# Corv/CUDA-GMM-MPI

Hardware: NVIDIA H100
Metric: EM iterations/sec at N=10M D=24 K=64; E-step HBM GB/s vs roofline (higher is better)
Workload: dtype f32

## Files before the change

cuda-gmm-mpi_b200/csrc/kernels_tc.cu:

```cuda
#include <cuda.h>
#include <cudaTypedefs.h>
#include <cuda_fp16.h>
#if defined(__F16C__) && defined(__AVX__)
#include <immintrin.h>
#endif
#include <cuda_runtime.h>

#include <cmath>
#include <cstdio>
#include <cstdlib>
#include <cstring>
#include <string>
#include <vector>

#include "host_math.h"
#include "kernels_tc.cuh"
#include "mstep_rows.h"
#include "tc_ptx.cuh"

namespace gmm {

using namespace ptx;

#define TC_CUDA_TRY(expr)                                                                     \
    do {                                                                                      \
        cudaError_t e_ = (expr);                                                              \
        if (e_ != cudaSuccess)                                                                \
            return fail(GMM_ERR_CUDA, std::string(#expr) + ": " + cudaGetErrorString(e_));    \
    } while (0)

constexpr int kTE = 32;
constexpr int kNCL = 32;
constexpr int kNST = 3;
constexpr int kNRAW = 4;
constexpr int kChunkSub = 4;
constexpr int kChunkSub2 = 16;
constexpr int kPhiBits = 11;
constexpr float kGammaScale = 1024.0f;
constexpr float kGammaMagic = 1.5f * 134217728.0f;

template <int D> struct MCfg {
    static_assert(D % 4 == 0, "tensor M-step: D must be a multiple of 4");
    static constexpr int F = 1 + D + D * (D + 1) / 2;
    static constexpr int S = D / 4;
    static constexpr int MT = (4 * ((1 + 2 * S + S * (D / 2) + 7) / 8) * 8 + 127) / 128;
    static constexpr int G_PART = kNCL * kTE * 2;
    static constexpr int G_STAGE = 3 * G_PART;
    static constexpr int RAWZ = (D * kTE * 4 + 1023) / 1024 * 1024;
    static constexpr int RAWX = RAWZ + 1024;
    static constexpr int RAWG = kNCL * kTE * 4;
    static constexpr int OFF_G = 0;
    static constexpr int OFF_RAWX = OFF_G + kNST * G_STAGE;
    static constexpr int OFF_RAWG = OFF_RAWX + kNRAW * RAWX;
    static constexpr int NCT = MT * 128;
    static constexpr int OFF_RACC = OFF_RAWG + kNRAW * RAWG;
    static constexpr int OFF_BAR = OFF_RACC + 32 * NCT * 4;
    static constexpr int SMEM_BYTES = OFF_BAR + 512;
    static constexpr int THREADS = 128 + NCT;
    static constexpr int REG_LAUNCH = (65536 / THREADS) / 8 * 8 > 255 ? 255 : (65536 / THREADS) / 8 * 8;
    static constexpr int REG_P = MT == 1 ? REG_LAUNCH : 56;
    static constexpr int REG_C = MT == 3 ? 152 : (MT == 2 ? 224 : REG_LAUNCH);
    static_assert(128 * REG_P + NCT * REG_C <= THREADS * REG_LAUNCH, "register pools");
    static_assert(OFF_RAWX % 1024 == 0 && RAWX % 1024 == 0 && RAWZ % 1024 == 0, "SWIZZLE_128B TMA destinations need 1024-byte alignment");
    static_assert(OFF_RAWG % 1024 == 0 && RAWG % 1024 == 0, "SWIZZLE_128B TMA destinations need 1024-byte alignment");
    static_assert(MT <= 3, "feature tiles");
};

template <int R, int L>
__device__ __forceinline__ void set_regs() {
    if constexpr (R < L) asm volatile("setmaxnreg.dec.sync.aligned.u32 %0;" ::"n"(R));
    else if constexpr (R > L) asm volatile("setmaxnreg.inc.sync.aligned.u32 %0;" ::"n"(R));
}

struct MMagic { float lin, prod; };

__device__ __forceinline__ void tma_load_2d(void* smem_dst, const CUtensorMap* tmap, int c0, int c1, uint64_t* bar) {
    asm volatile(
        "cp.async.bulk.tensor.2d.shared::cluster.global.mbarrier::complete_tx::bytes [%0], [%1, {%2, %3}], [%4];"
        ::"r"(smem_u32(smem_dst)), "l"(reinterpret_cast<uint64_t>(tmap)), "r"(c0), "r"(c1), "r"(smem_u32(bar)) : "memory");
}

__device__ __forceinline__ float2 lds_f2(uint32_t addr) {
    float2 v;
    asm volatile("ld.shared.v2.f32 {%0, %1}, [%2];" : "=f"(v.x), "=f"(v.y) : "r"(addr) : "memory");
    return v;
}

__device__ __forceinline__ void feature_split(float a, float b, float m, float& h, float& l) {
    h = __fsub_rn(__fmaf_rn(a, b, m), m);
    l = __fmaf_rn(a, b, -h);
}

#ifndef GMM_MSTEP_CUT
#define GMM_MSTEP_CUT 0
#endif

__device__ __forceinline__ void build_half(const float2 (&za)[4], const float2 (&zb0)[4], const float2 (&zb1)[4], float m0, float m1,
                                           uint32_t (&hi)[2][4], uint32_t (&lo)[2][4]) {
#pragma unroll
    for (int p = 0; p < 4; p++) {
        const int ks = p >> 1, u = p & 1;
#if GMM_MSTEP_CUT == 2
        hi[ks][2 * u] = __float_as_uint(zb0[p].x); hi[ks][2 * u + 1] = __float_as_uint(zb1[p].x);
        lo[ks][2 * u] = __float_as_uint(zb0[p].y); lo[ks][2 * u + 1] = __float_as_uint(zb1[p].y);
        (void)za; (void)m0; (void)m1;
#else
        float h0, l0, h1, l1, h2, l2, h3, l3;
        feature_split(za[p].x, zb0[p].x, m0, h0, l0);
        feature_split(za[p].y, zb0[p].y, m0, h1, l1);
        feature_split(za[p].x, zb1[p].x, m1, h2, l2);
        feature_split(za[p].y, zb1[p].y, m1, h3, l3);
        hi[ks][2 * u] = pack_half2(h0, h1);
        hi[ks][2 * u + 1] = pack_half2(h2, h3);
        lo[ks][2 * u] = pack_half2(l0, l1);
        lo[ks][2 * u + 1] = pack_half2(l2, l3);
#endif
    }
}

__device__ __forceinline__ void load_row(uint32_t addr, float2 (&z)[4]) {
#pragma unroll
    for (int p = 0; p < 4; p++) z[p] = lds_f2(addr ^ (uint32_t)(p << 5));
}

__device__ __forceinline__ void issue_half(float (&ex)[16], float (&rm)[16], const uint32_t (&hi)[2][4], const uint32_t (&lo)[2][4],
                                           uint32_t gam, bool new1, bool new2) {
#pragma unroll
    for (int ks = 0; ks < kTE / 16; ks++) {
        const uint64_t hdesc = make_smem_desc(gam + ks * 256,  128,  512);
        const uint64_t ldesc = make_smem_desc(gam + kNCL * kTE * 2 + ks * 256, 128, 512);
        const uint64_t sdesc = make_smem_desc(gam + 2 * kNCL * kTE * 2 + ks * 256, 128, 512);
#if GMM_MSTEP_CUT == 1
        asm volatile("" ::"r"(hi[ks][0]), "r"(hi[ks][1]), "r"(hi[ks][2]), "r"(hi[ks][3]), "r"(lo[ks][0]), "r"(lo[ks][1]), "r"(lo[ks][2]),
                     "r"(lo[ks][3]), "l"(hdesc), "l"(ldesc), "l"(sdesc));
        (void)ex; (void)rm; (void)new1; (void)new2;
#else
        wgmma_m64n32k16_rs(ex, hi[ks][0], hi[ks][1], hi[ks][2], hi[ks][3], hdesc, ks > 0 || !new1);
        wgmma_m64n32k16_rs(rm, hi[ks][0], hi[ks][1], hi[ks][2], hi[ks][3], ldesc, ks > 0 || !new2);
        wgmma_m64n32k16_rs(rm, lo[ks][0], lo[ks][1], lo[ks][2], lo[ks][3], sdesc, true);
#endif
    }
}

__device__ __forceinline__ bool chain_ends(int i, int mt, int nsub) { return ((i + mt) % kChunkSub) == kChunkSub - 1 || i == nsub - 1; }
__device__ __forceinline__ bool chain_starts(int i, int mt) { return i == 0 || ((i + mt) % kChunkSub) == 0; }
__device__ __forceinline__ bool chain2_ends(int i, int mt, int nsub) { return ((i + mt) % kChunkSub2) == kChunkSub2 - 1 || i == nsub - 1; }
__device__ __forceinline__ bool chain2_starts(int i, int mt) { return i == 0 || ((i + mt) % kChunkSub2) == 0; }

template <int D>
__global__ void __launch_bounds__(MCfg<D>::THREADS, 1)
mstep_tc_kernel(const __grid_constant__ CUtensorMap tm_x, const __grid_constant__ CUtensorMap tm_g, int n,
                float* __restrict__ scratch, int events_per_cta, const __grid_constant__ MMagic magic, const int* __restrict__ opmap) {
    using C = MCfg<D>;
    extern __shared__ __align__(1024) uint8_t smem[];
    uint64_t* bars = reinterpret_cast<uint64_t*>(smem + C::OFF_BAR);
    uint64_t* raw_full = bars;
    uint64_t* raw_empty = bars + kNRAW;
    uint64_t* op_full = bars + 2 * kNRAW;
    uint64_t* op_empty = op_full + kNST;

    const int warp = threadIdx.x >> 5, lane = threadIdx.x & 31;
    const int e_begin = blockIdx.x * events_per_cta;
    const int e_end = min(n, e_begin + events_per_cta);
    const int nsub = (e_end - e_begin + kTE - 1) / kTE;
    const int k0 = blockIdx.y * kNCL;

    for (int i = threadIdx.x; i < kNRAW * 256; i += C::THREADS)
        reinterpret_cast<float*>(smem + C::OFF_RAWX + (i >> 8) * C::RAWX + C::RAWZ)[i & 255] = 1.0f;
    if (threadIdx.x == 0) {
        for (int s = 0; s < kNRAW; s++) { mbar_init(&raw_full[s], 1); mbar_init(&raw_empty[s], 3 + 4 * C::MT); }
        for (int s = 0; s < kNST; s++) { mbar_init(&op_full[s], 3); mbar_init(&op_empty[s], 4 * C::MT); }
        fence_mbar_init();
    }
    __syncthreads();

    if (warp < 4) {
        set_regs<C::REG_P, C::REG_LAUNCH>();
        if (warp == 0) {
            if (elect_one()) {
                for (int i = 0; i < nsub; i++) {
                    const int st = i % kNRAW, ph = (i / kNRAW) & 1;
                    mbar_wait_parked(&raw_empty[st], ph ^ 1, 500);
                    mbar_arrive_expect_tx(&raw_full[st], kTE * D * 4 + C::RAWG);
                    const int e0 = e_begin + i * kTE;
                    tma_load_2d(smem + C::OFF_RAWX + st * C::RAWX, &tm_x, e0, 0, &raw_full[st]);
                    tma_load_2d(smem + C::OFF_RAWG + st * C::RAWG, &tm_g, e0, k0, &raw_full[st]);
                }
            }
        } else {
            const int bt = threadIdx.x - 32;
            constexpr int NIT = 2;
            for (int i = 0; i < nsub; i++) {
                const int rs = i % kNRAW, rph = (i / kNRAW) & 1;
                const int os = i % kNST, oph = (i / kNST) & 1;
                mbar_wait_parked(&raw_full[rs], rph, 200);
                uint4 gh[NIT], gl[NIT], gs[NIT];
                float dep = 0.0f;
#pragma unroll
                for (int u = 0; u < NIT; u++) {
                    const int it = bt + 96 * u;
                    if (it >= 128) break;
                    const int kg = it >> 5, l = it & 31;
                    const int k = kg * 8 + (l & 7), ce = l >> 3;
                    const uint8_t* grow = smem + C::OFF_RAWG + rs * C::RAWG + k * (kTE * 4);
                    const float4 a = *reinterpret_cast<const float4*>(grow + (((2 * ce) ^ (k & 7)) << 4));
                    const float4 b = *reinterpret_cast<const float4*>(grow + (((2 * ce + 1) ^ (k & 7)) << 4));
                    const float g[8] = {a.x, a.y, a.z, a.w, b.x, b.y, b.z, b.w};
                    dep += a.x + b.x;
                    float hi[8], lo[8];
#pragma unroll
                    for (int v = 0; v < 8; v++) {
                        hi[v] = __fsub_rn(__fmaf_rn(g[v], kGammaScale, kGammaMagic), kGammaMagic);
                        lo[v] = __fmaf_rn(g[v], kGammaScale, -hi[v]);
                    }
                    gh[u] = make_uint4(pack_half2(hi[0], hi[1]), pack_half2(hi[2], hi[3]), pack_half2(hi[4], hi[5]), pack_half2(hi[6], hi[7]));
                    gl[u] = make_uint4(pack_half2(lo[0], lo[1]), pack_half2(lo[2], lo[3]), pack_half2(lo[4], lo[5]), pack_half2(lo[6], lo[7]));
                    gs[u] = make_uint4(pack_half2(g[0] * kGammaScale, g[1] * kGammaScale), pack_half2(g[2] * kGammaScale, g[3] * kGammaScale),
                                       pack_half2(g[4] * kGammaScale, g[5] * kGammaScale), pack_half2(g[6] * kGammaScale, g[7] * kGammaScale));
                }
                __syncwarp();
                if (lane == 0) mbar_arrive_after(&raw_empty[rs], dep);
                else asm volatile("" ::"f"(dep));
                mbar_wait_parked(&op_empty[os], oph ^ 1, 200);
                uint8_t* g_hi = smem + C::OFF_G + os * C::G_STAGE;
#pragma unroll
                for (int u = 0; u < NIT; u++) {
                    const int it = bt + 96 * u;
                    if (it >= 128) break;
                    const int kg = it >> 5, l = it & 31;
                    *reinterpret_cast<uint4*>(g_hi + kg * 512 + l * 16) = gh[u];
                    *reinterpret_cast<uint4*>(g_hi + C::G_PART + kg * 512 + l * 16) = gl[u];
                    *reinterpret_cast<uint4*>(g_hi + 2 * C::G_PART + kg * 512 + l * 16) = gs[u];
                }
                fence_proxy_async_smem();
                __syncwarp();
                if (lane == 0) mbar_arrive(&op_full[os]);
            }
        }
    } else {
        set_regs<C::REG_C, C::REG_LAUNCH>();
        const int mt = __shfl_sync(0xffffffffu, (warp - 4) >> 2, 0);
        const int ct = threadIdx.x - 128;
        const int wq = warp & 3, gid = lane >> 2, qd = lane & 3;
        float* racc = reinterpret_cast<float*>(smem + C::OFF_RACC) + ct;
#pragma unroll
        for (int j = 0; j < 32; j++) racc[j * C::NCT] = 0.0f;
        uint32_t fa, fb[4];
        float mg[4];
        {
            const int* om = opmap + mt * 128 + wq * 16 + gid;
            auto addr = [&](int code) {
                const uint32_t row = code >= kRowOne ? (uint32_t)(C::RAWZ / 128 + code - kRowOne) : (uint32_t)code;
                return row * 128 + ((((uint32_t)qd >> 1) ^ (row & 7)) << 4) + ((uint32_t)qd & 1) * 8;
            };
#pragma unroll
            for (int s = 0; s < 4; s++) {
                const int c = om[(s >> 1) * 64 + (s & 1) * 8];
                const int a = c & 255, b = c >> 8;
                if (s == 0) fa = addr(a);
                fb[s] = addr(b);
                mg[s] = a >= kRowOne && b >= kRowOne ? 0.0f : (a >= kRowOne || b >= kRowOne ? magic.lin : magic.prod);
            }
        }
        const uint32_t zs0 = smem_u32(smem + C::OFF_RAWX);
        float ex[2][16], rm[2][16];
#pragma unroll
        for (int h = 0; h < 2; h++)
#pragma unroll
            for (int j = 0; j < 16; j++) { ex[h][j] = 0.0f; rm[h][j] = 0.0f; }
        uint32_t fh[2][2][4], fl[2][2][4];
        int held = -1;
        for (int i = 0; i < nsub; i++) {
            const int rs = i % kNRAW, rph = (i / kNRAW) & 1;
            const int os = i % kNST, oph = (i / kNST) & 1;
            const uint32_t zst = zs0 + rs * C::RAWX;
            const uint32_t gam = smem_u32(smem + C::OFF_G + os * C::G_STAGE);
            const bool new1 = chain_starts(i, mt), new2 = chain2_starts(i, mt);
            mbar_wait_parked(&raw_full[rs], rph, 100);
            float2 za[4], zb0[4], zb1[4];
            load_row(zst + fa, za);
            load_row(zst + fb[0], zb0);
            load_row(zst + fb[1], zb1);
            build_half(za, zb0, zb1, mg[0], mg[1], fh[0], fl[0]);
            mbar_wait_parked(&op_full[os], oph, 100);
            wgmma_fence();
            issue_half(ex[0], rm[0], fh[0], fl[0], gam, new1, new2);
            wgmma_commit();
            wgmma_wait<1>();
            __syncwarp();
            if (lane == 0 && held >= 0) mbar_arrive(&op_empty[held]);
            load_row(zst + fb[2], zb0);
            load_row(zst + fb[3], zb1);
            build_half(za, zb0, zb1, mg[2], mg[3], fh[1], fl[1]);
            wgmma_fence();
            issue_half(ex[1], rm[1], fh[1], fl[1], gam, new1, new2);
            wgmma_commit();
            __syncwarp();
            if (lane == 0) mbar_arrive(&raw_empty[rs]);
            wgmma_wait<1>();
            held = os;
            if (chain_ends(i, mt, nsub)) {
                wgmma_wait<0>();
                __syncwarp();
                if (lane == 0) mbar_arrive(&op_empty[os]);
                held = -1;
#if GMM_MSTEP_CUT != 3
#pragma unroll
                for (int h = 0; h < 2; h++) {
#pragma unroll
                    for (int j = 0; j < 16; j++) racc[(h * 16 + j) * C::NCT] += ex[h][j];
                    asm volatile("" ::: "memory");
                }
                if (chain2_ends(i, mt, nsub)) {
#pragma unroll
                    for (int h = 0; h < 2; h++) {
#pragma unroll
                        for (int j = 0; j < 16; j++) racc[(h * 16 + j) * C::NCT] += rm[h][j];
                        asm volatile("" ::: "memory");
                    }
                }
#endif
            }
        }
        wgmma_wait<0>();
#if GMM_MSTEP_CUT == 3
#pragma unroll
        for (int h = 0; h < 2; h++)
#pragma unroll
            for (int j = 0; j < 16; j++) racc[(h * 16 + j) * C::NCT] += ex[h][j] + rm[h][j];
#endif
        float* my = scratch + (size_t)(blockIdx.y * gridDim.x + blockIdx.x) * C::MT * 128 * kNCL + (size_t)mt * 128 * kNCL;
#pragma unroll
        for (int h = 0; h < 2; h++)
#pragma unroll
            for (int j = 0; j < 16; j += 2) {
                const int row = h * 64 + wq * 16 + gid + 8 * ((j >> 1) & 1);
                const int col = (j >> 2) * 8 + 2 * qd;
                *reinterpret_cast<float2*>(my + (size_t)row * kNCL + col) =
                    make_float2(racc[(h * 16 + j) * C::NCT], racc[(h * 16 + j + 1) * C::NCT]);
            }
    }
}

__global__ void standardise_soa_kernel(const float* __restrict__ xs, float* __restrict__ zs, size_t pitch, int n, int D,
                                       const float* __restrict__ shift_f, const float* __restrict__ inv_scale_f) {
    const int d = blockIdx.y;
    const float s = shift_f[d], isc = inv_scale_f[d];
    const float* x = xs + (size_t)d * pitch;
    float* z = zs + (size_t)d * pitch;
    for (long long e = (long long)blockIdx.x * blockDim.x + threadIdx.x; e < n; e += (long long)gridDim.x * blockDim.x)
        z[e] = __fmul_rn(__fsub_rn(x[e], s), isc);
}

__global__ void __launch_bounds__(256)
mstep_tc_finalize_kernel(const float* __restrict__ scratch, int ncta_x, int MT, int K, int F, const int3* __restrict__ rowmap,
                         const double* __restrict__ scale, double* __restrict__ stats) {
    constexpr int NQ = 256 / kNCL;
    __shared__ double part[NQ][kNCL];
    const int3 rm = rowmap[blockIdx.x];
    if (rm.x < 0) return;
    const int mt = blockIdx.x / 128, row = blockIdx.x % 128;
    const int col = threadIdx.x & (kNCL - 1), q = threadIdx.x / kNCL;
    double fac = 1.0 / (double)kGammaScale;
    if (rm.y >= 0) fac *= scale[rm.y];
    if (rm.z >= 0) fac *= scale[rm.z];
    for (int ty = 0; ty * kNCL < K; ty++) {
        double s = 0;
        for (int cx = q; cx < ncta_x; cx += NQ)
            s += (double)scratch[(((size_t)(ty * ncta_x + cx) * MT + mt) * 128 + row) * kNCL + col];
        part[q][col] = s;
        __syncthreads();
        const int k = ty * kNCL + col;
        if (q == 0 && k < K) {
            double t = 0;
#pragma unroll
            for (int u = 0; u < NQ; u++) t += part[u][col];
            stats[(size_t)k * F + rm.x] += t * fac;
        }
        __syncthreads();
    }
}


template <int D> struct ECfg {
    static_assert(D % 8 == 0, "tensor E-step: D must be a multiple of 8");
    static constexpr int CP = D / 8;
    static constexpr int NLO = (CP + 1 + 1) / 2 * 2;
    static constexpr int NCHKB = CP + NLO;
    static constexpr int GB = 16;
    static constexpr int N = GB * 8;
    static constexpr int MAXSG = 64 / GB;
    static constexpr int B_BLOCK = NCHKB * N * 16;
    static constexpr int B_SG = CP * B_BLOCK;
    static constexpr int OFF_B = 0;
    static constexpr int OFF_CK = OFF_B + MAXSG * B_SG;
    static constexpr int OFF_SH = OFF_CK + 512;
    static constexpr int OFF_BAR = OFF_SH + 256;
    static constexpr int SMEM_BYTES = OFF_BAR + 64;
    static constexpr int NWG = 2;
    static constexpr int THREADS = 128 * NWG;
};

#ifndef GMM_ESTEP_CUT
#define GMM_ESTEP_CUT 0
#endif

template <int D>
__device__ __forceinline__ void tc_stage_operand(uint8_t* smem, const uint8_t* __restrict__ b_img, const float* __restrict__ ck,
                                                 const float* __restrict__ shift_f, const float* __restrict__ inv_scale_f, int NSG) {
    using C = ECfg<D>;
    uint64_t* b_full = reinterpret_cast<uint64_t*>(smem + C::OFF_BAR);
    float* ck_s = reinterpret_cast<float*>(smem + C::OFF_CK);
    float* sh_s = reinterpret_cast<float*>(smem + C::OFF_SH);
    if (threadIdx.x == 0) { mbar_init(b_full, 1); fence_mbar_init(); }
    if (threadIdx.x < 64) { ck_s[threadIdx.x] = ck[threadIdx.x] * 1.4426950408889634f; ck_s[64 + threadIdx.x] = ck[64 + threadIdx.x]; }
    if (threadIdx.x < D) { sh_s[threadIdx.x] = shift_f[threadIdx.x]; sh_s[32 + threadIdx.x] = inv_scale_f[threadIdx.x]; }
    __syncthreads();
    if (threadIdx.x == 0) {
        mbar_arrive_expect_tx(b_full, (uint32_t)NSG * C::B_SG);
        for (int g = 0; g < NSG * C::CP; g++) tma_load_1d(smem + C::OFF_B + g * C::B_BLOCK, b_img + (size_t)g * C::B_BLOCK, C::B_BLOCK, b_full);
    }
}
// ... 418 lines not shown
        if (cudaGetDriverEntryPoint("cuTensorMapEncodeTiled", &p, cudaEnableDefault, &q) == cudaSuccess && q == cudaDriverEntryPointSuccess)
            fn = reinterpret_cast<PFN_cuTensorMapEncodeTiled_v12000>(p);
    }
    return fn;
}

static int make_map_2d(CUtensorMap* m, const void* base, uint64_t dim0, uint64_t dim1, uint64_t stride1_bytes, uint32_t box0, uint32_t box1,
                       bool swizzle128 = false) {
    auto fn = encode_fn();
    if (!fn) return fail(GMM_ERR_CUDA, "cuTensorMapEncodeTiled not available from the driver");
    cuuint64_t dims[2] = {dim0, dim1};
    cuuint64_t strides[1] = {stride1_bytes};
    cuuint32_t box[2] = {box0, box1};
    cuuint32_t estr[2] = {1, 1};
    CUresult r = fn(m, CU_TENSOR_MAP_DATA_TYPE_FLOAT32, 2, const_cast<void*>(base), dims, strides, box, estr,
                    CU_TENSOR_MAP_INTERLEAVE_NONE, swizzle128 ? CU_TENSOR_MAP_SWIZZLE_128B : CU_TENSOR_MAP_SWIZZLE_NONE, CU_TENSOR_MAP_L2_PROMOTION_L2_128B,
                    CU_TENSOR_MAP_FLOAT_OOB_FILL_NONE);
    if (r != CUDA_SUCCESS) return fail(GMM_ERR_CUDA, "cuTensorMapEncodeTiled failed (" + std::to_string((int)r) + ")");
    return GMM_OK;
}

bool tc_mstep_supported(int D, int K) {
    (void)K;
    return D == 4 || D == 8 || D == 12 || D == 16 || D == 20 || D == 24;
}
bool tc_estep_supported(int D, int K) { return (D == 8 || D == 16 || D == 24) && K >= 1 && K <= GMM_MAX_CLUSTERS; }

template <int D> static size_t ecfg_pass_bytes() { return (size_t)ECfg<D>::MAXSG * ECfg<D>::B_SG; }
static size_t pass_bytes_for(int D) {
    switch (D) { case 8: return ecfg_pass_bytes<8>(); case 16: return ecfg_pass_bytes<16>(); case 24: return ecfg_pass_bytes<24>(); default: return 0; }
}

int tc_create(TcState** out, const float* d_x_aos, const float* d_x_soa, int n, int D, int Kmax, float* d_memb, size_t memb_pitch, int num_sms,
              cudaStream_t stream) {
    (void)stream;
    TcState* t = new TcState();
    t->d_x = d_x_aos; t->d_x_soa = d_x_soa; t->d_memb = d_memb; t->memb_pitch = memb_pitch; t->n = n; t->D = D; t->Kmax = Kmax; t->num_sms = num_sms;
    *out = t;
    if (n <= 0 || !tc_mstep_supported(D, Kmax)) return GMM_OK;
    TC_CUDA_TRY(cudaMalloc(&t->d_shift_f, sizeof(float) * GMM_MAX_DIMENSIONS));
    TC_CUDA_TRY(cudaMalloc(&t->d_inv_scale_f, sizeof(float) * GMM_MAX_DIMENSIONS));
    TC_CUDA_TRY(cudaMalloc(&t->d_scale, sizeof(double) * GMM_MAX_DIMENSIONS));
    TC_CUDA_TRY(cudaMalloc(&t->d_z_soa, sizeof(float) * memb_pitch * D));
    if (int rc = make_map_2d(&t->tm_x, t->d_z_soa, (uint64_t)n, (uint64_t)D, (uint64_t)memb_pitch * 4, kTE, (uint32_t)D, true)) return rc;
    if (int rc = make_map_2d(&t->tm_g, d_memb, (uint64_t)n, (uint64_t)Kmax, (uint64_t)memb_pitch * 4, kTE, kNCL, true)) return rc;
    t->maps_ok = true;
    if (D == 8 || D == 16 || D == 24) {
        const int passes = (Kmax + 63) / 64;
        t->e_ck_len = passes * 64;
        t->bimg_bytes = (size_t)passes * pass_bytes_for(D);
        const size_t ck_bytes = sizeof(float) * 2 * t->e_ck_len;
        TC_CUDA_TRY(cudaMalloc(&t->d_opnd, ck_bytes + t->bimg_bytes));
        TC_CUDA_TRY(cudaMallocHost(&t->h_opnd, ck_bytes + t->bimg_bytes));
        t->d_ck = reinterpret_cast<float*>(t->d_opnd);
        t->h_ck = reinterpret_cast<float*>(t->h_opnd);
        t->d_bimg = t->d_opnd + ck_bytes;
        t->h_bimg = t->h_opnd + ck_bytes;
        TC_CUDA_TRY(cudaEventCreateWithFlags(&t->ev_h2d, cudaEventDisableTiming));
        if (passes > 1) TC_CUDA_TRY(cudaMalloc(&t->d_den, sizeof(float) * memb_pitch));
        t->emap_ok = true;
    }
    const int mt = mstep_tiles(D);
    {
        const std::vector<MRow> rows = mstep_row_layout(D);
        if (rows.size() != (size_t)mt * 128) return fail(GMM_ERR_STATE, "tensor M-step row map: the statistics do not fit the feature tiles");
        std::vector<int3> rm(rows.size());
        std::vector<int> om(rows.size());
        std::vector<char> seen((size_t)num_features(D), 0);
        for (size_t row = 0; row < rows.size(); row++) {
            const MRow& r = rows[row];
            rm[row] = make_int3(r.f, r.i, r.j);
            om[row] = r.a | r.b << 8;
            if (r.f >= 0) {
                if (seen[r.f]) return fail(GMM_ERR_STATE, "tensor M-step row map: a statistic is produced twice");
                seen[r.f] = 1;
            }
        }
        for (char c : seen) if (!c) return fail(GMM_ERR_STATE, "tensor M-step row map: a statistic is not produced");
        TC_CUDA_TRY(cudaMalloc(&t->d_rowmap, sizeof(int3) * rm.size()));
        TC_CUDA_TRY(cudaMemcpy(t->d_rowmap, rm.data(), sizeof(int3) * rm.size(), cudaMemcpyHostToDevice));
        TC_CUDA_TRY(cudaMalloc(&t->d_opmap, sizeof(int) * om.size()));
        TC_CUDA_TRY(cudaMemcpy(t->d_opmap, om.data(), sizeof(int) * om.size(), cudaMemcpyHostToDevice));
    }
    const int ytiles = (Kmax + kNCL - 1) / kNCL;
    t->scratch_floats = (size_t)num_sms * ytiles * mt * 128 * kNCL;
    TC_CUDA_TRY(cudaMalloc(&t->d_scratch, sizeof(float) * t->scratch_floats));
    return GMM_OK;
}

void tc_set_host_threads(TcState* t, int n) { if (t) t->host_threads = n < 1 ? 1 : n; }
bool tc_mstep_ready(const TcState* t) { return t && t->maps_ok && t->have_shift && t->mstep_ready; }
bool tc_estep_range_ok(const TcState* t) {
    if (!t || !t->have_shift) return false;
    for (int d = 0; d < t->D; d++)
        if (!(t->zmax[d] <= 16384.0f)) return false;
    return true;
}

void tc_destroy(TcState* t) {
    if (!t) return;
    cudaFree(t->d_shift_f); cudaFree(t->d_inv_scale_f); cudaFree(t->d_scale); cudaFree(t->d_scratch);
    cudaFree(t->d_opnd); cudaFree(t->d_den); cudaFree(t->d_z_soa); cudaFree(t->d_rowmap); cudaFree(t->d_opmap);
    if (t->h_opnd) cudaFreeHost(t->h_opnd);
    if (t->ev_h2d) cudaEventDestroy(t->ev_h2d);
    delete t;
}

int tc_set_shift_scale(TcState* t, double* shift, const double* scale, const double* xmin, const double* xmax, cudaStream_t stream) {
    if (!t || !t->maps_ok) return GMM_OK;
    float sf[GMM_MAX_DIMENSIONS] = {0}, isf[GMM_MAX_DIMENSIONS] = {0};
    double sc[GMM_MAX_DIMENSIONS] = {0};
    for (int d = 0; d < t->D; d++) {
        sf[d] = (float)shift[d];
        shift[d] = (double)sf[d];
        const double s = (scale && scale[d] > 0) ? scale[d] : 1.0;
        isf[d] = (float)(1.0 / s);
        sc[d] = 1.0 / (double)isf[d];
        t->h_shift[d] = shift[d];
        t->h_scale[d] = sc[d];
        const double za = std::fmax(std::fabs(xmax[d] - (double)sf[d]), std::fabs(xmin[d] - (double)sf[d])) * (double)isf[d] * (1.0 + 1e-6);
        int e2 = 0;
        if (za > 0 && std::isfinite(za)) { e2 = std::ilogb(za) + 1; }
        t->zmax[d] = std::isfinite(za) ? (float)std::ldexp(1.0, e2) : INFINITY;
    }
    {
        float zb = 0.f;
        for (int d = 0; d < t->D; d++) zb = std::fmax(zb, t->zmax[d]);
        t->mstep_ready = zb <= 64.0f;
        const double q = (double)zb / (double)(1 << kPhiBits);
        t->magic.lin = (float)(1.5 * 8388608.0 * q);
        t->magic.prod = (float)(1.5 * 8388608.0 * q * (double)zb);
    }
    TC_CUDA_TRY(cudaMemcpyAsync(t->d_shift_f, sf, sizeof(sf), cudaMemcpyHostToDevice, stream));
    TC_CUDA_TRY(cudaMemcpyAsync(t->d_inv_scale_f, isf, sizeof(isf), cudaMemcpyHostToDevice, stream));
    TC_CUDA_TRY(cudaMemcpyAsync(t->d_scale, sc, sizeof(sc), cudaMemcpyHostToDevice, stream));
    {
        dim3 grid((unsigned)std::min<long long>(4LL * t->num_sms, ((long long)t->n + 255) / 256), (unsigned)t->D);
        standardise_soa_kernel<<<grid, 256, 0, stream>>>(t->d_x_soa, t->d_z_soa, t->memb_pitch, t->n, t->D, t->d_shift_f, t->d_inv_scale_f);
        TC_CUDA_TRY(cudaGetLastError());
    }
    TC_CUDA_TRY(cudaStreamSynchronize(stream));
    t->have_shift = true;
    return GMM_OK;
}


static inline uint16_t f2h_bits(float f) {
    uint32_t x;
    std::memcpy(&x, &f, 4);
    const uint32_t sign = (x >> 16) & 0x8000u;
    x &= 0x7fffffffu;
    if (x >= 0x47800000u) return (uint16_t)(sign | 0x7c00u);
    if (x < 0x38800000u) {
        float a;
        std::memcpy(&a, &x, 4);
        return (uint16_t)(sign | (uint32_t)lrintf(a * 16777216.0f));
    }
    x += ((x >> 13) & 1u) + 0xfffu;
    return (uint16_t)(sign | ((x - 0x38000000u) >> 13));
}
static inline float h2f_bits(uint16_t h) {
    const uint32_t sign = (uint32_t)(h & 0x8000u) << 16;
    const uint32_t em = h & 0x7fffu;
    float r;
    if (em >= 0x0400u) {
        const uint32_t x = sign | ((em << 13) + 0x38000000u);
        std::memcpy(&r, &x, 4);
// ... 411 lines not shown
    const int ntiles = (n + 127) / 128;
    int grid = t->num_sms;
    if (grid > ntiles) grid = ntiles;
    if (grid < 1) grid = 1;
    const int NP = (K + 63) / 64;
    if (NP > 1 && !den) return fail(GMM_ERR_STATE, "tensor E-step: context was created for at most 64 clusters");
    auto launch = [&](int p, int mode, const float* den_in, float* den_out) {
        const int Kp = K - 64 * p < 64 ? K - 64 * p : 64;
        kern[(Kp + C::GB - 1) / C::GB - 1]<<<grid, C::THREADS, C::SMEM_BYTES, stream>>>(
            x, t->d_bimg + (size_t)p * C::MAXSG * C::B_SG, t->d_ck + 128 * p, t->d_shift_f, t->d_inv_scale_f,
            memb + (size_t)(64 * p) * pitch, pitch, n, Kp, d_ll, mode, den_in, den_out);
        return cudaGetLastError();
    };
    if (NP == 1) TC_CUDA_TRY(launch(0, 0, nullptr, nullptr));
    else {
        for (int p = 0; p + 1 < NP; p++) TC_CUDA_TRY(launch(p, 1, p ? den : nullptr, den));
        TC_CUDA_TRY(launch(NP - 1, 2, den, den));
        for (int p = 0; p + 1 < NP; p++) TC_CUDA_TRY(launch(p, 3, den, nullptr));
    }
    return GMM_OK;
}

static int launch_estep_any(TcState* t, int K, const float* x, int n, float* memb, size_t pitch, float* den, double* d_ll, cudaStream_t stream) {
    if (!t || !t->emap_ok) return fail(GMM_ERR_STATE, "tensor E-step not initialised for this shape");
    switch (t->D) {
        case 8: return launch_estep_d<8>(t, K, x, n, memb, pitch, den, d_ll, stream);
        case 16: return launch_estep_d<16>(t, K, x, n, memb, pitch, den, d_ll, stream);
        case 24: return launch_estep_d<24>(t, K, x, n, memb, pitch, den, d_ll, stream);
        default: return fail(GMM_ERR_ARG, "tensor E-step: unsupported D");
    }
}

int tc_launch_estep(TcState* t, int K, double* d_ll, cudaStream_t stream) {
    if (!t) return fail(GMM_ERR_STATE, "tensor E-step not initialised for this shape");
    return launch_estep_any(t, K, t->d_x, t->n, t->d_memb, t->memb_pitch, t->d_den, d_ll, stream);
}

int tc_launch_estep_on(TcState* t, int K, const float* d_x_aos, int n, float* d_memb, size_t pitch, float* d_den, double* d_ll,
                       cudaStream_t stream) {
    if (n <= 0) return GMM_OK;
    return launch_estep_any(t, K, d_x_aos, n, d_memb, pitch, d_den, d_ll, stream);
}

template <int D>
static int launch_score_d(TcState* t, int K, const TcScoreIo& io, cudaStream_t stream) {
    using C = ECfg<D>;
    static void (*const kern[C::MAXSG])(const float*, const uint8_t*, const float*, const float*, const float*, int, int, int, int, int,
                                        float*, float*, int*, int*, float*, float*, double*, int*) = {
        score_tc_kernel<D, 1>, score_tc_kernel<D, 2>, score_tc_kernel<D, 3>, score_tc_kernel<D, 4>};
    static_assert(C::MAXSG == 4, "one kernel instance per supergroup count");
    if (!t->attr_score) {
        for (auto* k : kern) TC_CUDA_TRY(cudaFuncSetAttribute(k, cudaFuncAttributeMaxDynamicSharedMemorySize, C::SMEM_BYTES));
        t->attr_score = true;
    }
    const int ntiles = (io.n + 127) / 128;
    int grid = t->num_sms;
    if (grid > ntiles) grid = ntiles;
    if (grid < 1) grid = 1;
    const int NP = (K + 63) / 64;
    if (NP > 1 && !(io.run_den && io.run_bl && io.run_bk)) return fail(GMM_ERR_STATE, "tensor scoring: no running state for K > 64");
    for (int p = 0; p < NP; p++) {
        const int Kp = K - 64 * p < 64 ? K - 64 * p : 64;
        kern[(Kp + C::GB - 1) / C::GB - 1]<<<grid, C::THREADS, C::SMEM_BYTES, stream>>>(
            io.x, t->d_bimg + (size_t)p * C::MAXSG * C::B_SG, t->d_ck + 128 * p, t->d_shift_f, t->d_inv_scale_f, io.n, Kp, 64 * p, p, p + 1 == NP, io.run_den, io.run_bl, io.run_bk, io.labels, io.max_resp, io.logp, io.ll,
            io.flag);
        TC_CUDA_TRY(cudaGetLastError());
    }
    return GMM_OK;
}

int tc_launch_score(TcState* t, int K, const TcScoreIo& io, cudaStream_t stream) {
    if (!t || !t->emap_ok) return fail(GMM_ERR_STATE, "tensor scoring not initialised for this shape");
    if (io.n <= 0) return GMM_OK;
    switch (t->D) {
        case 8: return launch_score_d<8>(t, K, io, stream);
        case 16: return launch_score_d<16>(t, K, io, stream);
        case 24: return launch_score_d<24>(t, K, io, stream);
        default: return fail(GMM_ERR_ARG, "tensor scoring: unsupported D");
    }
}

template <int D>
static int launch_mstep_d(TcState* t, int K, const CUtensorMap& tm_x, const CUtensorMap& tm_g, int n, double* d_stats, cudaStream_t stream) {
    using C = MCfg<D>;
    static_assert(C::SMEM_BYTES <= 232448, "shared memory budget");
    if (!t->attr_mstep) {
        TC_CUDA_TRY(cudaFuncSetAttribute(mstep_tc_kernel<D>, cudaFuncAttributeMaxDynamicSharedMemorySize, C::SMEM_BYTES));
        t->attr_mstep = true;
    }
    int gx = t->num_sms;
    int per = (n + gx - 1) / gx;
    per = (per + kTE - 1) / kTE * kTE;
    gx = (n + per - 1) / per;
    const int gy = (K + kNCL - 1) / kNCL;
    if ((size_t)gx * gy * C::MT * 128 * kNCL > t->scratch_floats) return fail(GMM_ERR_STATE, "tensor M-step scratch too small");
    dim3 grid(gx, gy);
    mstep_tc_kernel<D><<<grid, C::THREADS, C::SMEM_BYTES, stream>>>(tm_x, tm_g, n, t->d_scratch, per, t->magic, t->d_opmap);
    TC_CUDA_TRY(cudaGetLastError());
    mstep_tc_finalize_kernel<<<C::MT * 128, 256, 0, stream>>>(t->d_scratch, gx, C::MT, K, C::F, t->d_rowmap, t->d_scale, d_stats);
    TC_CUDA_TRY(cudaGetLastError());
    return GMM_OK;
}

static int launch_mstep_any(TcState* t, int K, const CUtensorMap& tm_x, const CUtensorMap& tm_g, int n, double* d_stats, cudaStream_t stream) {
    if (!t || !t->maps_ok) return fail(GMM_ERR_STATE, "tensor-core M-step not initialised for this shape");
    if (!t->have_shift) return fail(GMM_ERR_STATE, "tensor-core M-step needs gmm_seed (shift/scale) first");
    if (!t->mstep_ready) return fail(GMM_ERR_STATE, "tensor-core M-step: the data range exceeds the fixed-point operand budget");
    switch (t->D) {
        case 4: return launch_mstep_d<4>(t, K, tm_x, tm_g, n, d_stats, stream);
        case 8: return launch_mstep_d<8>(t, K, tm_x, tm_g, n, d_stats, stream);
        case 12: return launch_mstep_d<12>(t, K, tm_x, tm_g, n, d_stats, stream);
        case 16: return launch_mstep_d<16>(t, K, tm_x, tm_g, n, d_stats, stream);
        case 20: return launch_mstep_d<20>(t, K, tm_x, tm_g, n, d_stats, stream);
        case 24: return launch_mstep_d<24>(t, K, tm_x, tm_g, n, d_stats, stream);
        default: return fail(GMM_ERR_ARG, "tensor-core M-step: unsupported D");
    }
}

int tc_launch_mstep(TcState* t, int K, double* d_stats, cudaStream_t stream) {
    if (!t) return fail(GMM_ERR_STATE, "tensor-core M-step not initialised for this shape");
    return launch_mstep_any(t, K, t->tm_x, t->tm_g, t->n, d_stats, stream);
}

int tc_launch_mstep_on(TcState* t, int K, const float* d_z, const float* d_memb, size_t pitch, int n, double* d_stats, cudaStream_t stream) {
    if (n <= 0) return GMM_OK;
    if (!t || !t->maps_ok) return fail(GMM_ERR_STATE, "tensor-core M-step not initialised for this shape");
    if (t->cmap_z != d_z || t->cmap_g != d_memb || t->cmap_pitch != pitch || t->cmap_n != n) {
        t->cmap_n = -1;
        if (int rc = make_map_2d(&t->tm_cx, d_z, (uint64_t)n, (uint64_t)t->D, (uint64_t)pitch * 4, kTE, (uint32_t)t->D, true)) return rc;
        if (int rc = make_map_2d(&t->tm_cg, d_memb, (uint64_t)n, (uint64_t)t->Kmax, (uint64_t)pitch * 4, kTE, kNCL, true)) return rc;
        t->cmap_z = d_z; t->cmap_g = d_memb; t->cmap_pitch = pitch; t->cmap_n = n;
    }
    return launch_mstep_any(t, K, t->tm_cx, t->tm_cg, n, d_stats, stream);
}

const float* tc_shift_f(const TcState* t) { return t && t->have_shift ? t->d_shift_f : nullptr; }
const float* tc_inv_scale_f(const TcState* t) { return t && t->have_shift ? t->d_inv_scale_f : nullptr; }
float tc_mstep_zbound(const TcState* t) {
    float zb = 0.f;
    if (t)
        for (int d = 0; d < t->D; d++) zb = std::fmax(zb, t->zmax[d]);
    return zb;
}

}
```

Before: 126.5.

## Widen tensor M-step CTA to 64 clusters, splitting feature half-tiles across paired CTAs

Result: faster. 136.2 (median of 6 runs) (+7.7%).

```diff
diff --git a/cuda-gmm-mpi_b200/csrc/kernels_tc.cu b/cuda-gmm-mpi_b200/csrc/kernels_tc.cu
--- a/cuda-gmm-mpi_b200/csrc/kernels_tc.cu
+++ b/cuda-gmm-mpi_b200/csrc/kernels_tc.cu
@@ -11,6 +11,7 @@
 #include <cstdlib>
 #include <cstring>
 #include <string>
+#include <type_traits>
 #include <vector>
 
 #include "host_math.h"
@@ -39,16 +40,19 @@
 constexpr float kGammaScale = 1024.0f;
 constexpr float kGammaMagic = 1.5f * 134217728.0f;
 
-template <int D> struct MCfg {
+template <int D, int NCL_> struct MCfg {
     static_assert(D % 4 == 0, "tensor M-step: D must be a multiple of 4");
+    static_assert(NCL_ == 32 || NCL_ == 64, "tensor M-step: 32 or 64 clusters per CTA");
+    static constexpr int NCL = NCL_;
+    static constexpr int HPC = 64 / NCL;
     static constexpr int F = 1 + D + D * (D + 1) / 2;
     static constexpr int S = D / 4;
     static constexpr int MT = (4 * ((1 + 2 * S + S * (D / 2) + 7) / 8) * 8 + 127) / 128;
-    static constexpr int G_PART = kNCL * kTE * 2;
+    static constexpr int G_PART = NCL * kTE * 2;
     static constexpr int G_STAGE = 3 * G_PART;
     static constexpr int RAWZ = (D * kTE * 4 + 1023) / 1024 * 1024;
     static constexpr int RAWX = RAWZ + 1024;
-    static constexpr int RAWG = kNCL * kTE * 4;
+    static constexpr int RAWG = NCL * kTE * 4;
     static constexpr int OFF_G = 0;
     static constexpr int OFF_RAWX = OFF_G + kNST * G_STAGE;
     static constexpr int OFF_RAWG = OFF_RAWX + kNRAW * RAWX;
@@ -123,21 +127,28 @@
     for (int p = 0; p < 4; p++) z[p] = lds_f2(addr ^ (uint32_t)(p << 5));
 }
 
-__device__ __forceinline__ void issue_half(float (&ex)[16], float (&rm)[16], const uint32_t (&hi)[2][4], const uint32_t (&lo)[2][4],
+template <int NCL>
+__device__ __forceinline__ void issue_half(float (&ex)[NCL / 2], float (&rm)[NCL / 2], const uint32_t (&hi)[2][4], const uint32_t (&lo)[2][4],
                                            uint32_t gam, bool new1, bool new2) {
 #pragma unroll
     for (int ks = 0; ks < kTE / 16; ks++) {
         const uint64_t hdesc = make_smem_desc(gam + ks * 256,  128,  512);
-        const uint64_t ldesc = make_smem_desc(gam + kNCL * kTE * 2 + ks * 256, 128, 512);
-        const uint64_t sdesc = make_smem_desc(gam + 2 * kNCL * kTE * 2 + ks * 256, 128, 512);
+        const uint64_t ldesc = make_smem_desc(gam + NCL * kTE * 2 + ks * 256, 128, 512);
+        const uint64_t sdesc = make_smem_desc(gam + 2 * NCL * kTE * 2 + ks * 256, 128, 512);
 #if GMM_MSTEP_CUT == 1
         asm volatile("" ::"r"(hi[ks][0]), "r"(hi[ks][1]), "r"(hi[ks][2]), "r"(hi[ks][3]), "r"(lo[ks][0]), "r"(lo[ks][1]), "r"(lo[ks][2]),
                      "r"(lo[ks][3]), "l"(hdesc), "l"(ldesc), "l"(sdesc));
         (void)ex; (void)rm; (void)new1; (void)new2;
 #else
-        wgmma_m64n32k16_rs(ex, hi[ks][0], hi[ks][1], hi[ks][2], hi[ks][3], hdesc, ks > 0 || !new1);
-        wgmma_m64n32k16_rs(rm, hi[ks][0], hi[ks][1], hi[ks][2], hi[ks][3], ldesc, ks > 0 || !new2);
-        wgmma_m64n32k16_rs(rm, lo[ks][0], lo[ks][1], lo[ks][2], lo[ks][3], sdesc, true);
+        if constexpr (NCL == 32) {
+            wgmma_m64n32k16_rs(ex, hi[ks][0], hi[ks][1], hi[ks][2], hi[ks][3], hdesc, ks > 0 || !new1);
+            wgmma_m64n32k16_rs(rm, hi[ks][0], hi[ks][1], hi[ks][2], hi[ks][3], ldesc, ks > 0 || !new2);
+            wgmma_m64n32k16_rs(rm, lo[ks][0], lo[ks][1], lo[ks][2], lo[ks][3], sdesc, true);
+        } else {
+            wgmma_m64n64k16_rs(ex, hi[ks][0], hi[ks][1], hi[ks][2], hi[ks][3], hdesc, ks > 0 || !new1);
+            wgmma_m64n64k16_rs(rm, hi[ks][0], hi[ks][1], hi[ks][2], hi[ks][3], ldesc, ks > 0 || !new2);
+            wgmma_m64n64k16_rs(rm, lo[ks][0], lo[ks][1], lo[ks][2], lo[ks][3], sdesc, true);
+        }
 #endif
     }
 }
@@ -147,11 +158,12 @@
 __device__ __forceinline__ bool chain2_ends(int i, int mt, int nsub) { return ((i + mt) % kChunkSub2) == kChunkSub2 - 1 || i == nsub - 1; }
 __device__ __forceinline__ bool chain2_starts(int i, int mt) { return i == 0 || ((i + mt) % kChunkSub2) == 0; }
 
-template <int D>
-__global__ void __launch_bounds__(MCfg<D>::THREADS, 1)
-mstep_tc_kernel(const __grid_constant__ CUtensorMap tm_x, const __grid_constant__ CUtensorMap tm_g, int n,
+template <int D, int NCL>
+__global__ void __launch_bounds__(MCfg<D, NCL>::THREADS, 1)
+mstep_tc_kernel(const __grid_constant__ CUtensorMap tm_x, const __grid_constant__ CUtensorMap tm_g, int n, int K,
                 float* __restrict__ scratch, int events_per_cta, const __grid_constant__ MMagic magic, const int* __restrict__ opmap) {
-    using C = MCfg<D>;
+    using C = MCfg<D, NCL>;
+    constexpr int HPC = C::HPC;
     extern __shared__ __align__(1024) uint8_t smem[];
     uint64_t* bars = reinterpret_cast<uint64_t*>(smem + C::OFF_BAR);
     uint64_t* raw_full = bars;
@@ -160,10 +172,11 @@
     uint64_t* op_empty = op_full + kNST;
 
     const int warp = threadIdx.x >> 5, lane = threadIdx.x & 31;
-    const int e_begin = blockIdx.x * events_per_cta;
+    const int range = blockIdx.x / (2 / HPC), part = blockIdx.x % (2 / HPC);
+    const int e_begin = range * events_per_cta;
     const int e_end = min(n, e_begin + events_per_cta);
     const int nsub = (e_end - e_begin + kTE - 1) / kTE;
-    const int k0 = blockIdx.y * kNCL;
+    const int k0 = blockIdx.y * NCL;
 
     for (int i = threadIdx.x; i < kNRAW * 256; i += C::THREADS)
         reinterpret_cast<float*>(smem + C::OFF_RAWX + (i >> 8) * C::RAWX + C::RAWZ)[i & 255] = 1.0f;
@@ -177,29 +190,32 @@
     if (warp < 4) {
         set_regs<C::REG_P, C::REG_LAUNCH>();
         if (warp == 0) {
+            const int nbox = min(NCL, K - k0 + kNCL - 1) / kNCL;
             if (elect_one()) {
                 for (int i = 0; i < nsub; i++) {
                     const int st = i % kNRAW, ph = (i / kNRAW) & 1;
                     mbar_wait_parked(&raw_empty[st], ph ^ 1, 500);
-                    mbar_arrive_expect_tx(&raw_full[st], kTE * D * 4 + C::RAWG);
+                    mbar_arrive_expect_tx(&raw_full[st], kTE * D * 4 + nbox * kNCL * kTE * 4);
                     const int e0 = e_begin + i * kTE;
                     tma_load_2d(smem + C::OFF_RAWX + st * C::RAWX, &tm_x, e0, 0, &raw_full[st]);
-                    tma_load_2d(smem + C::OFF_RAWG + st * C::RAWG, &tm_g, e0, k0, &raw_full[st]);
+                    for (int b = 0; b < nbox; b++)
+                        tma_load_2d(smem + C::OFF_RAWG + st * C::RAWG + b * kNCL * kTE * 4, &tm_g, e0, k0 + b * kNCL, &raw_full[st]);
                 }
             }
         } else {
             const int bt = threadIdx.x - 32;
-            constexpr int NIT = 2;
+            constexpr int NITEM = 4 * NCL, NIT = (NITEM + 95) / 96;
             for (int i = 0; i < nsub; i++) {
                 const int rs = i % kNRAW, rph = (i / kNRAW) & 1;
                 const int os = i % kNST, oph = (i / kNST) & 1;
                 mbar_wait_parked(&raw_full[rs], rph, 200);
-                uint4 gh[NIT], gl[NIT], gs[NIT];
+                mbar_wait_parked(&op_empty[os], oph ^ 1, 200);
+                uint8_t* g_hi = smem + C::OFF_G + os * C::G_STAGE;
                 float dep = 0.0f;
 #pragma unroll
                 for (int u = 0; u < NIT; u++) {
                     const int it = bt + 96 * u;
-                    if (it >= 128) break;
+                    if (it >= NITEM) break;
                     const int kg = it >> 5, l = it & 31;
                     const int k = kg * 8 + (l & 7), ce = l >> 3;
                     const uint8_t* grow = smem + C::OFF_RAWG + rs * C::RAWG + k * (kTE * 4);
@@ -213,25 +229,17 @@
                         hi[v] = __fsub_rn(__fmaf_rn(g[v], kGammaScale, kGammaMagic), kGammaMagic);
                         lo[v] = __fmaf_rn(g[v], kGammaScale, -hi[v]);
                     }
-                    gh[u] = make_uint4(pack_half2(hi[0], hi[1]), pack_half2(hi[2], hi[3]), pack_half2(hi[4], hi[5]), pack_half2(hi[6], hi[7]));
-                    gl[u] = make_uint4(pack_half2(lo[0], lo[1]), pack_half2(lo[2], lo[3]), pack_half2(lo[4], lo[5]), pack_half2(lo[6], lo[7]));
-                    gs[u] = make_uint4(pack_half2(g[0] * kGammaScale, g[1] * kGammaScale), pack_half2(g[2] * kGammaScale, g[3] * kGammaScale),
-                                       pack_half2(g[4] * kGammaScale, g[5] * kGammaScale), pack_half2(g[6] * kGammaScale, g[7] * kGammaScale));
+                    *reinterpret_cast<uint4*>(g_hi + kg * 512 + l * 16) =
+                        make_uint4(pack_half2(hi[0], hi[1]), pack_half2(hi[2], hi[3]), pack_half2(hi[4], hi[5]), pack_half2(hi[6], hi[7]));
+                    *reinterpret_cast<uint4*>(g_hi + C::G_PART + kg * 512 + l * 16) =
+                        make_uint4(pack_half2(lo[0], lo[1]), pack_half2(lo[2], lo[3]), pack_half2(lo[4], lo[5]), pack_half2(lo[6], lo[7]));
+                    *reinterpret_cast<uint4*>(g_hi + 2 * C::G_PART + kg * 512 + l * 16) =
+                        make_uint4(pack_half2(g[0] * kGammaScale, g[1] * kGammaScale), pack_half2(g[2] * kGammaScale, g[3] * kGammaScale),
+                                   pack_half2(g[4] * kGammaScale, g[5] * kGammaScale), pack_half2(g[6] * kGammaScale, g[7] * kGammaScale));
                 }
                 __syncwarp();
                 if (lane == 0) mbar_arrive_after(&raw_empty[rs], dep);
                 else asm volatile("" ::"f"(dep));
-                mbar_wait_parked(&op_empty[os], oph ^ 1, 200);
-                uint8_t* g_hi = smem + C::OFF_G + os * C::G_STAGE;
-#pragma unroll
-                for (int u = 0; u < NIT; u++) {
-                    const int it = bt + 96 * u;
-                    if (it >= 128) break;
-                    const int kg = it >> 5, l = it & 31;
-                    *reinterpret_cast<uint4*>(g_hi + kg * 512 + l * 16) = gh[u];
-                    *reinterpret_cast<uint4*>(g_hi + C::G_PART + kg * 512 + l * 16) = gl[u];
-                    *reinterpret_cast<uint4*>(g_hi + 2 * C::G_PART + kg * 512 + l * 16) = gs[u];
-                }
                 fence_proxy_async_smem();
                 __syncwarp();
                 if (lane == 0) mbar_arrive(&op_full[os]);
@@ -239,22 +247,25 @@
         }
     } else {
         set_regs<C::REG_C, C::REG_LAUNCH>();
-        const int mt = __shfl_sync(0xffffffffu, (warp - 4) >> 2, 0);
+        const int cw = __shfl_sync(0xffffffffu, (warp - 4) >> 2, 0);
+        const int hx = HPC == 2 ? 2 * cw : part * C::MT + cw;
+        const int mt = hx >> 1;
         const int ct = threadIdx.x - 128;
         const int wq = warp & 3, gid = lane >> 2, qd = lane & 3;
         float* racc = reinterpret_cast<float*>(smem + C::OFF_RACC) + ct;
 #pragma unroll
         for (int j = 0; j < 32; j++) racc[j * C::NCT] = 0.0f;
-        uint32_t fa, fb[4];
-        float mg[4];
+        constexpr int NSLOT = 2 * HPC;
+        uint32_t fa, fb[NSLOT];
+        float mg[NSLOT];
         {
-            const int* om = opmap + mt * 128 + wq * 16 + gid;
+            const int* om = opmap + hx * 64 + wq * 16 + gid;
             auto addr = [&](int code) {
                 const uint32_t row = code >= kRowOne ? (uint32_t)(C::RAWZ / 128 + code - kRowOne) : (uint32_t)code;
                 return row * 128 + ((((uint32_t)qd >> 1) ^ (row & 7)) << 4) + ((uint32_t)qd & 1) * 8;
             };
 #pragma unroll
-            for (int s = 0; s < 4; s++) {
+            for (int s = 0; s < NSLOT; s++) {
                 const int c = om[(s >> 1) * 64 + (s & 1) * 8];
                 const int a = c & 255, b = c >> 8;
                 if (s == 0) fa = addr(a);
@@ -263,81 +274,101 @@
             }
         }
         const uint32_t zs0 = smem_u32(smem + C::OFF_RAWX);
-        float ex[2][16], rm[2][16];
-#pragma unroll
-        for (int h = 0; h < 2; h++)
-#pragma unroll
-            for (int j = 0; j < 16; j++) { ex[h][j] = 0.0f; rm[h][j] = 0.0f; }
+        float ex[HPC][NCL / 2], rm[HPC][NCL / 2];
+#pragma unroll
+        for (int h = 0; h < HPC; h++)
+#pragma unroll
+            for (int j = 0; j < NCL / 2; j++) { ex[h][j] = 0.0f; rm[h][j] = 0.0f; }
+        auto add_to_racc = [&](float (&acc)[HPC][NCL / 2]) {
+#pragma unroll
+            for (int c = 0; c < 2; c++) {
+#pragma unroll
+                for (int j = 0; j < 16; j++) {
+                    const int q = 16 * c + j;
+                    racc[q * C::NCT] += acc[q / (NCL / 2)][q % (NCL / 2)];
+                }
+                asm volatile("" ::: "memory");
+            }
+        };
         uint32_t fh[2][2][4], fl[2][2][4];
+        float2 za[4];
         int held = -1;
-        for (int i = 0; i < nsub; i++) {
+        auto group = [&](int i, auto hc, uint32_t (&gh)[2][4], uint32_t (&gl)[2][4]) {
+            constexpr int h = decltype(hc)::value;
             const int rs = i % kNRAW, rph = (i / kNRAW) & 1;
             const int os = i % kNST, oph = (i / kNST) & 1;
             const uint32_t zst = zs0 + rs * C::RAWX;
             const uint32_t gam = smem_u32(smem + C::OFF_G + os * C::G_STAGE);
             const bool new1 = chain_starts(i, mt), new2 = chain2_starts(i, mt);
-            mbar_wait_parked(&raw_full[rs], rph, 100);
-            float2 za[4], zb0[4], zb1[4];
-            load_row(zst + fa, za);
-            load_row(zst + fb[0], zb0);
-            load_row(zst + fb[1], zb1);
-            build_half(za, zb0, zb1, mg[0], mg[1], fh[0], fl[0]);
-            mbar_wait_parked(&op_full[os], oph, 100);
+            if constexpr (h == 0) {
+                mbar_wait_parked(&raw_full[rs], rph, 100);
+                load_row(zst + fa, za);
+            }
+            float2 zb0[4], zb1[4];
+            load_row(zst + fb[2 * h], zb0);
+            load_row(zst + fb[2 * h + 1], zb1);
+            build_half(za, zb0, zb1, mg[2 * h], mg[2 * h + 1], gh, gl);
+            if constexpr (h == 0) mbar_wait_parked(&op_full[os], oph, 100);
             wgmma_fence();
-            issue_half(ex[0], rm[0], fh[0], fl[0], gam, new1, new2);
+            issue_half<NCL>(ex[h], rm[h], gh, gl, gam, new1, new2);
             wgmma_commit();
+            if constexpr (h == HPC - 1) {
+                __syncwarp();
+                if (lane == 0) mbar_arrive(&raw_empty[rs]);
+            }
             wgmma_wait<1>();
-            __syncwarp();
-            if (lane == 0 && held >= 0) mbar_arrive(&op_empty[held]);
-            load_row(zst + fb[2], zb0);
-            load_row(zst + fb[3], zb1);
-            build_half(za, zb0, zb1, mg[2], mg[3], fh[1], fl[1]);
-            wgmma_fence();
-            issue_half(ex[1], rm[1], fh[1], fl[1], gam, new1, new2);
-            wgmma_commit();
-            __syncwarp();
-            if (lane == 0) mbar_arrive(&raw_empty[rs]);
-            wgmma_wait<1>();
-            held = os;
-            if (chain_ends(i, mt, nsub)) {
-                wgmma_wait<0>();
+            if constexpr (h == 0) {
                 __syncwarp();
-                if (lane == 0) mbar_arrive(&op_empty[os]);
-                held = -1;
+                if (lane == 0 && held >= 0) mbar_arrive(&op_empty[held]);
+            }
+            if constexpr (h == HPC - 1) {
+                held = os;
+                if (chain_ends(i, mt, nsub)) {
+                    wgmma_wait<0>();
+                    __syncwarp();
+                    if (lane == 0) mbar_arrive(&op_empty[os]);
+                    held = -1;
 #if GMM_MSTEP_CUT != 3
-#pragma unroll
-                for (int h = 0; h < 2; h++) {
-#pragma unroll
-                    for (int j = 0; j < 16; j++) racc[(h * 16 + j) * C::NCT] += ex[h][j];
-                    asm volatile("" ::: "memory");
+                    add_to_racc(ex);
+                    if (chain2_ends(i, mt, nsub)) add_to_racc(rm);
+#endif
                 }
-                if (chain2_ends(i, mt, nsub)) {
-#pragma unroll
-                    for (int h = 0; h < 2; h++) {
-#pragma unroll
-                        for (int j = 0; j < 16; j++) racc[(h * 16 + j) * C::NCT] += rm[h][j];
-                        asm volatile("" ::: "memory");
-                    }
-                }
-#endif
-            }
+            }
+        };
+        using H0 = std::integral_constant<int, 0>;
+        using H1 = std::integral_constant<int, 1>;
+        if constexpr (HPC == 2) {
+            for (int i = 0; i < nsub; i++) {
+                group(i, H0{}, fh[0], fl[0]);
+                group(i, H1{}, fh[1], fl[1]);
+            }
+        } else {
+            int i = 0;
+            for (; i + 1 < nsub; i += 2) {
+                group(i, H0{}, fh[0], fl[0]);
+                group(i + 1, H0{}, fh[1], fl[1]);
+            }
+            if (i < nsub) group(i, H0{}, fh[0], fl[0]);
         }
         wgmma_wait<0>();
 #if GMM_MSTEP_CUT == 3
 #pragma unroll
-        for (int h = 0; h < 2; h++)
-#pragma unroll
-            for (int j = 0; j < 16; j++) racc[(h * 16 + j) * C::NCT] += ex[h][j] + rm[h][j];
+        for (int h = 0; h < HPC; h++)
+#pragma unroll
+            for (int j = 0; j < NCL / 2; j++) ex[h][j] += rm[h][j];
+        add_to_racc(ex);
 #endif
-        float* my = scratch + (size_t)(blockIdx.y * gridDim.x + blockIdx.x) * C::MT * 128 * kNCL + (size_t)mt * 128 * kNCL;
-#pragma unroll
-        for (int h = 0; h < 2; h++)
-#pragma unroll
-            for (int j = 0; j < 16; j += 2) {
-                const int row = h * 64 + wq * 16 + gid + 8 * ((j >> 1) & 1);
+        const int nranges = gridDim.x * HPC / 2;
+#pragma unroll
+        for (int h = 0; h < HPC; h++)
+#pragma unroll
+            for (int j = 0; j < NCL / 2; j += 2) {
+                const int q = h * (NCL / 2) + j;
+                const int row = ((hx & 1) + h) * 64 + wq * 16 + gid + 8 * ((j >> 1) & 1);
                 const int col = (j >> 2) * 8 + 2 * qd;
-                *reinterpret_cast<float2*>(my + (size_t)row * kNCL + col) =
-                    make_float2(racc[(h * 16 + j) * C::NCT], racc[(h * 16 + j + 1) * C::NCT]);
+                const int ty = blockIdx.y * (NCL / kNCL) + col / kNCL;
+                float* dst = scratch + ((((size_t)ty * nranges + range) * C::MT + mt) * 128 + row) * kNCL + col % kNCL;
+                *reinterpret_cast<float2*>(dst) = make_float2(racc[q * C::NCT], racc[(q + 1) * C::NCT]);
             }
     }
 }
@@ -922,7 +953,7 @@
         TC_CUDA_TRY(cudaMalloc(&t->d_opmap, sizeof(int) * om.size()));
         TC_CUDA_TRY(cudaMemcpy(t->d_opmap, om.data(), sizeof(int) * om.size(), cudaMemcpyHostToDevice));
     }
-    const int ytiles = (Kmax + kNCL - 1) / kNCL;
+    const int ytiles = (Kmax + 63) / 64 * (64 / kNCL);
     t->scratch_floats = (size_t)num_sms * ytiles * mt * 128 * kNCL;
     TC_CUDA_TRY(cudaMalloc(&t->d_scratch, sizeof(float) * t->scratch_floats));
     return GMM_OK;
@@ -1500,22 +1531,28 @@
 
 template <int D>
 static int launch_mstep_d(TcState* t, int K, const CUtensorMap& tm_x, const CUtensorMap& tm_g, int n, double* d_stats, cudaStream_t stream) {
-    using C = MCfg<D>;
-    static_assert(C::SMEM_BYTES <= 232448, "shared memory budget");
+    using C32 = MCfg<D, 32>;
+    using C64 = MCfg<D, 64>;
+    static_assert(C32::SMEM_BYTES <= 232448 && C64::SMEM_BYTES <= 232448, "shared memory budget");
     if (!t->attr_mstep) {
-        TC_CUDA_TRY(cudaFuncSetAttribute(mstep_tc_kernel<D>, cudaFuncAttributeMaxDynamicSharedMemorySize, C::SMEM_BYTES));
+        TC_CUDA_TRY(cudaFuncSetAttribute(mstep_tc_kernel<D, 32>, cudaFuncAttributeMaxDynamicSharedMemorySize, C32::SMEM_BYTES));
+        TC_CUDA_TRY(cudaFuncSetAttribute(mstep_tc_kernel<D, 64>, cudaFuncAttributeMaxDynamicSharedMemorySize, C64::SMEM_BYTES));
         t->attr_mstep = true;
     }
     int gx = t->num_sms;
     int per = (n + gx - 1) / gx;
     per = (per + kTE - 1) / kTE * kTE;
     gx = (n + per - 1) / per;
-    const int gy = (K + kNCL - 1) / kNCL;
-    if ((size_t)gx * gy * C::MT * 128 * kNCL > t->scratch_floats) return fail(GMM_ERR_STATE, "tensor M-step scratch too small");
-    dim3 grid(gx, gy);
-    mstep_tc_kernel<D><<<grid, C::THREADS, C::SMEM_BYTES, stream>>>(tm_x, tm_g, n, t->d_scratch, per, t->magic, t->d_opmap);
+    const bool pair = K > 32;
+    const int ncl = pair ? 64 : 32;
+    const int gy = (K + ncl - 1) / ncl;
+    if ((size_t)gx * gy * (ncl / kNCL) * C32::MT * 128 * kNCL > t->scratch_floats) return fail(GMM_ERR_STATE, "tensor M-step scratch too small");
+    if (pair)
+        mstep_tc_kernel<D, 64><<<dim3(2 * gx, gy), C64::THREADS, C64::SMEM_BYTES, stream>>>(tm_x, tm_g, n, K, t->d_scratch, per, t->magic, t->d_opmap);
+    else
+        mstep_tc_kernel<D, 32><<<dim3(gx, gy), C32::THREADS, C32::SMEM_BYTES, stream>>>(tm_x, tm_g, n, K, t->d_scratch, per, t->magic, t->d_opmap);
     TC_CUDA_TRY(cudaGetLastError());
-    mstep_tc_finalize_kernel<<<C::MT * 128, 256, 0, stream>>>(t->d_scratch, gx, C::MT, K, C::F, t->d_rowmap, t->d_scale, d_stats);
+    mstep_tc_finalize_kernel<<<C32::MT * 128, 256, 0, stream>>>(t->d_scratch, gx, C32::MT, K, C32::F, t->d_rowmap, t->d_scale, d_stats);
     TC_CUDA_TRY(cudaGetLastError());
     return GMM_OK;
 }
```
